# icadriani/nn_conformer_for_speech_recognition

Measured on AMD Instinct MI355X. Metric: mel-frames/sec/GPU Conformer-L encoder fwd+bwd; 1/2/4/8-GPU scaling, higher is better.
Workload: dtype bf16; 1 GPU; Conformer-L encoder fwd+bwd + CTC head, 32 x 15 s utterances per GPU; model=Conformer-L, layers=17, d_model=512, heads=8, ffn=2048, conv_kernel=31, pos_enc=none, specaug=False, global_batch=32, seq_len=1501, enc_frames=373, frontend=frame, optimizer=adafactor, parallelism=dp1, launch=hip-graph (fwd+bwd), grad_reduce_dtype=fp32

## Files before the change

### include/cfm.h

```cpp
#ifndef CFM_H
#define CFM_H

#include <stddef.h>
#include <stdint.h>

#ifdef __cplusplus
extern "C" {
#endif

#define CFM_F32 0
#define CFM_BF16 1
#define CFM_FP8 2

#define CFM_OK 0
#define CFM_ERR_ARG (-1)
#define CFM_ERR_SHAPE (-2)
#define CFM_ERR_DTYPE (-3)
#define CFM_ERR_ALIGN (-4)
#define CFM_ERR_UNSUPPORTED (-5)
#define CFM_ERR_LAUNCH (-6)

#define CFM_ACT_NONE 0
#define CFM_ACT_SILU 1

// ... 218 lines not shown
int cfm_bn_silu_bwd(const void* dz, int dtype_dz, const float* y, const float* gamma,
                    const float* beta, const float* mean, const float* invstd, int training,
                    float* dy, float* dgamma, float* dbeta, long M, int C, float* ws, void* stream);
int cfm_bn_silu_fwd_sums(const float* ws, int B, int T, int C, float* sums, void* stream);
int cfm_bn_silu_fwd_apply(const float* y, const float* gamma, const float* beta, float* running_mean,
                          float* running_var, float momentum, float eps, const float* sums, long M_total, float* mean,
                          float* invstd, void* z, int dtz, long M, int C, void* stream);
int cfm_bn_silu_bwd_sums(const void* dz, int dtdz, const float* y, const float* gamma, const float* beta,
                         const float* mean, const float* invstd, long M, int C, float* ws, float* dbeta, float* dgamma,
                         void* stream);
int cfm_bn_silu_bwd_apply(const void* dz, int dtdz, const float* y, const float* gamma, const float* beta,
                          const float* mean, const float* invstd, const float* dbeta_total, const float* dgamma_total,
                          long M_total, float* dy, long M, int C, void* stream);
size_t cfm_bn_ws_bytes(int C);
int cfm_bn_fwd(const float* y, const float* gamma, const float* beta, float* running_mean,
               float* running_var, float momentum, float eps, int training, float* mean, float* invstd,
               void* z, int dtype_z, long M, int C, int act, float* ws, void* stream);
int cfm_bn_bwd(const void* dz, int dtype_dz, const float* y, const float* gamma, const float* beta,
               const float* mean, const float* invstd, int training, int act, float* dy, float* dgamma,
               float* dbeta, long M, int C, float* ws, void* stream);
int cfm_glu_dwconv_bwd(const float* dy, const void* a, int dtype_a, const float* w_dw, void* da,
                       int dtype_da, float* dw, float* db, int B, int T, int C, int K, float* ws,
                       void* stream);
int cfm_glu_dwconv_bwd_wgrad(float* ws, int B, int T, int C, int K, float* dw, float* db, void* stream);
int cfm_glu_dwconv_bwd_bn(const void* dz, int dtype_dz, const float* y, const float* gamma, const float* beta,
                          const float* mean, const float* invstd, const float* dbeta, const float* dgamma,
                          float invM, int training, const void* a, int dtype_a, const float* w_dw, void* da,
                          int dtype_da, float* dw, float* db, int B, int T, int C, int K, float* ws, void* stream);
int cfm_gn_silu_fwd(const float* y, const float* gamma, const float* beta, float eps, float* mean, float* rstd,
                    void* z, int dtype_z, int B, int T, int C, const float* ws, void* stream);
int cfm_gn_silu_bwd_sums(const void* dz, int dtype_dz, const float* y, const float* gamma, const float* beta,
                         const float* mean, const float* rstd, int B, int T, int C, float* ws, float* dbeta,
                         float* dgamma, float* coef, void* stream);
int cfm_glu_dwconv_bwd_gn(const void* dz, int dtype_dz, const float* y, const float* gamma, const float* beta,
                          const float* mean, const float* rstd, const float* coef, const void* a, int dtype_a,
                          const float* w_dw, void* da, int dtype_da, float* dw, float* db, int B, int T, int C, int K,
                          float* ws, void* stream);
int cfm_gn_silu_bwd(const void* dz, int dtype_dz, const float* y, const float* gamma, const float* beta,
                    const float* mean, const float* rstd, float* dy, float* dgamma, float* dbeta, float* coef,
                    int B, int T, int C, float* ws, void* stream);

enum cfm_convmod_op {
  CFM_CONVMOD_OP_FWD = 0,
  CFM_CONVMOD_OP_BWD = 1,
  CFM_CONVMOD_OP_BWD_BN = 2,
  CFM_CONVMOD_OP_BWD_GN = 3
};
enum cfm_convmod_family {
  CFM_CONVMOD_FAM_UNSUPPORTED = 0,
  CFM_CONVMOD_FAM_VEC = 1,
  CFM_CONVMOD_FAM_SCALAR_KT = 2,
  CFM_CONVMOD_FAM_SCALAR_KRT = 3
};
enum cfm_convmod_apply {
  CFM_CONVMOD_APPLY_NONE = 0,
  CFM_CONVMOD_APPLY_SCALAR = 1,
  CFM_CONVMOD_APPLY_VEC8 = 2
};
typedef struct {
  int op;
  int norm;
  int dtype_a, dtype_da, dtype_dz, dtype_z;
  long M;
  int C, K;
  const void* y;
  const void* z;
  int force_scalar;
} cfm_convmod_query;
typedef struct {
  int family;
  int dz16;
  int apply;
} cfm_convmod_choice;
int cfm_convmod_plan(const cfm_convmod_query* q, cfm_convmod_choice* out);

enum cfm_attn_mode {
  CFM_ATTN_MODE_TILED = 1 << 0,
  CFM_ATTN_MODE_STAGING_ONLY = 1 << 1,
  CFM_ATTN_MODE_SKIP_STORES = 1 << 2,
  CFM_ATTN_MODE_REL_SIMT = 1 << 4,
  CFM_ATTN_MODE_REL_ZERO_FILL = 1 << 6,
  CFM_ATTN_MODE_REL_DPOS_R4 = 1 << 7,
  CFM_ATTN_MODE_REL_DQ_RECOMPUTE = 1 << 9,
  CFM_ATTN_MODE_DQ_RECOMPUTE = 1 << 10
};
int cfm_attn_set_mode(int mode);

enum cfm_attn_path {
  CFM_ATTN_PATH_SIMT = 0,
  CFM_ATTN_PATH_HEAD = 1,
  CFM_ATTN_PATH_TILED = 2,
  CFM_ATTN_PATH_REL = 3
};
enum cfm_attn_dpos {
  CFM_ATTN_DPOS_NONE = 0,
  CFM_ATTN_DPOS_XCD = 1,
  CFM_ATTN_DPOS_R4_VEC = 2,
  CFM_ATTN_DPOS_R4 = 3
};
enum cfm_attn_ws {
  CFM_ATTN_WS_D = 0,
  CFM_ATTN_WS_PART = 1,
  CFM_ATTN_WS_DS = 2,
  CFM_ATTN_WS_DPOS = 3
};
typedef struct {
  int B, T, H, dk, dtype;
  int rel;
  int qkv_mod16, dout_mod16, pos_mod16;
  int mode;
  int cus;
  int64_t ws_bytes;
} cfm_attn_query;
typedef struct {
  int path;
  int vec, vec4;
  int pvec, rel_vec;
  int dbg;
  int qs, waves;
  int dq_stored;
  int dpos;
  size_t lds_head, lds_dkdv, lds_dqs;
  size_t ws_off[4], ws_size[4];
  size_t ws_total;
} cfm_attn_choice;
int cfm_attn_plan(const cfm_attn_query* q, cfm_attn_choice* out);

int cfm_attn_fwd(const void* qkv, void* o, float* lse, const int32_t* lengths, const void* pos,
                 const float* pos_u, const float* pos_v, int B, int T, int H, int dk, int dtype,
                 float drop_p, uint64_t seed, void* stream);
size_t cfm_attn_bwd_ws_bytes(int B, int T, int H, int dk, int rel, int dtype);
int cfm_attn_bwd(const void* qkv, const void* o, const void* dout, const float* lse,
                 const int32_t* lengths, const void* pos, const float* pos_u, const float* pos_v,
                 void* dqkv, float* dpos, float* dpos_u, float* dpos_v, int B, int T, int H,
                 int dk, int dtype, float drop_p, uint64_t seed, float* ws, size_t ws_bytes, void* stream);
int cfm_attn_bwd_ex(const void* qkv, const void* o, const void* dout, const float* lse,
                    const int32_t* lengths, const void* pos, const float* pos_u, const float* pos_v,
                    void* dqkv, void* dpos, int dtype_dpos, float* dpos_u, float* dpos_v, int B, int T,
                    int H, int dk, int dtype, float drop_p, uint64_t seed, int d_ready, float* ws,
                    size_t ws_bytes, void* stream);

int cfm_conv1_fwd(const float* x, const float* w1, const float* b1, void* h1, int dtype_h, int B,
                  int F, int T, int C1, void* stream);
int cfm_conv2_fwd(const void* h1, const void* w2r, const float* b2, void* h2, int dtype_h2,
                  int dtype, int B, int F1, int T1, int C1, int C2, void* stream);
int cfm_conv2_bwd_data(const void* dh2, const void* w2r, void* dh1, int dtype, int B, int F1,
                       int T1, int C1, int C2, void* stream);
size_t cfm_conv2_bwd_data_ws_bytes(int C1, int C2);
int cfm_conv2_bwd_data_ws(const void* dh2, const void* w2r, void* dh1, int dtype, int B, int F1,
                          int T1, int C1, int C2, void* ws, void* stream);
int cfm_conv2_bwd_weight(const void* dh2, const void* h1, float* dw2r, int dtype, int B, int F1,
                         int T1, int C1, int C2, void* stream);
size_t cfm_conv2_bwd_weight_ws_bytes(int B, int F1, int T1, int C1, int C2);
int cfm_conv2_bwd_weight_ws(const void* dh2, const void* h1, float* dw2r, int dtype, int B, int F1,
                            int T1, int C1, int C2, float* ws, void* stream);
size_t cfm_conv1_bwd_ws_bytes(int B, int F, int T, int C1);
int cfm_conv1_bwd_weight(const void* dh1, int dtype_h, const float* x, float* dw1, float* db1,
                         int B, int F, int T, int C1, float* ws, void* stream);

typedef struct {
  int B, F, T;
  int C1, C2, D;
  int k1, s1, k2, s2;
  int dtype;
  int hilo;
  int F2, T2, Ke, Se, Fp, Cx, Kp, lda, T2p, Tslot;
  long xt_elems;
// ... 95 lines not shown
```

### nn_conformer_for_speech_recognition_amd/_lib.py

```python
from __future__ import annotations

import ctypes
import os
import subprocess

import torch

_HERE = os.path.dirname(os.path.abspath(__file__))
LIB_PATH = os.environ.get("CFM_LIB") or os.path.join(_HERE, "libcfm.so")
CSRC = os.path.join(_HERE, "csrc")

F32, BF16, FP8 = 0, 1, 2
ACT_NONE, ACT_SILU = 0, 1

c_void_p, c_int, c_long, c_float, c_size_t = ctypes.c_void_p, ctypes.c_int, ctypes.c_long, ctypes.c_float, ctypes.c_size_t
c_u64 = ctypes.c_uint64


class NGramLMDesc(ctypes.Structure):
    _fields_ = [("unigrams", c_void_p), ("table", c_void_p), ("seed", c_u64), ("mask", ctypes.c_uint32),
                ("probe", c_int), ("order", c_int), ("V", c_int)]


class GemmDesc(ctypes.Structure):
    _fields_ = [
        ("M", c_int), ("N", c_int), ("K", c_int), ("batch", c_int),
        ("dtype_ab", c_int),
        ("A", c_void_p), ("lda", c_long), ("stride_a", c_long), ("a_kmajor", c_int),
        ("B", c_void_p), ("ldb", c_long), ("stride_b", c_long), ("b_kmajor", c_int),
        ("C", c_void_p), ("ldc", c_long), ("stride_c", c_long), ("dtype_c", c_int),
        ("alpha", c_float),
        ("bias", c_void_p),
        ("act", c_int),
        ("act_grad", c_int),
        ("pre", c_void_p), ("dtype_pre", c_int),
        ("drop_p", c_float), ("drop_seed", c_u64), ("drop_offset", c_u64),
        ("out_scale", c_float),
        ("residual", c_void_p), ("ldr", c_long), ("dtype_r", c_int),
        ("split_k", c_int),
        ("workspace", c_void_p),
        ("probe", c_void_p),
        ("a_colsum", c_void_p),
        ("rowdot_with", c_void_p), ("rowdot_out", c_void_p), ("rowdot_T", c_int),
        ("alpha_a_dev", c_void_p), ("alpha_b_dev", c_void_p),
        ("allow_overlap", c_int),
        ("mx_a", c_void_p), ("mx_b", c_void_p),
        ("mx_out", c_void_p), ("mx_out_scales", c_void_p),
    ]


class GemmChoice(ctypes.Structure):
    _fields_ = [("variant", c_int), ("epilogue", c_int), ("grid_x", ctypes.c_uint), ("grid_y", ctypes.c_uint),
                ("grid_z", ctypes.c_uint), ("block", ctypes.c_uint)]


GEMM_MODE_STAGED256 = 1 << 0
GEMM_MODE_PIPE = 1 << 1
GEMM_MODE_DEFAULT = 3
GEMM_MODE_SKIP_STORES = 1 << 3
GEMM_MODE_SEL_SHIFT = 4
GEMM_MODE_SEL_MASK = 7 << 4
GEMM_MODE_GENERIC_DROPOUT = 1 << 10
GEMM_MODE_NO_192S8_RULE = 1 << 12
GEMM_MODE_SKIP_MAINLOOP = 1 << 13
GEMM_MODE_GENERIC_EPILOGUE = 1 << 14
GEMM_MODE_KEEP_SHARED_DMA = 1 << 19
GEMM_MODE_KEEP_PIPE192 = 1 << 21
GEMM_MODE_KEEP_128WIDE = 1 << 22
GEMM_MODE_KEEP_WS192 = 1 << 23
GEMM_SEL_AUTO, GEMM_SEL_PIPE256, GEMM_SEL_PIPE256S, GEMM_SEL_192, GEMM_SEL_PIPE192S8 = 0, 1, 2, 5, 7
(GEMM_V_NONE, GEMM_V_STAGED_BF16_256, GEMM_V_STAGED_BF16_128, GEMM_V_STAGED_F32_128, GEMM_V_STAGED_F32_64,
 GEMM_V_PIPE64X160, GEMM_V_WS192, GEMM_V_WS96, GEMM_V_PIPE192, GEMM_V_PIPE192S8, GEMM_V_PIPE256, GEMM_V_PIPE256S,
 GEMM_V_FP8_192, GEMM_V_FP8_256S, GEMM_V_MX192, GEMM_V_MX256S) = range(16)
(GEMM_EPI_GENERIC, GEMM_EPI_BF16, GEMM_EPI_BF16_BIAS, GEMM_EPI_BF16_SILU, GEMM_EPI_BF16_ACTG, GEMM_EPI_BF16_RD,
 GEMM_EPI_F32, GEMM_EPI_F32_RES, GEMM_EPI_BF16_SILU_MX, GEMM_EPI_BF16_RES, GEMM_EPI_F32R_BF16,
 GEMM_EPI_BF16_DELTA) = range(12)
CONVMOD_OP_FWD, CONVMOD_OP_BWD, CONVMOD_OP_BWD_BN, CONVMOD_OP_BWD_GN = range(4)
CONVMOD_FAM_UNSUPPORTED, CONVMOD_FAM_VEC, CONVMOD_FAM_SCALAR_KT, CONVMOD_FAM_SCALAR_KRT = range(4)
CONVMOD_APPLY_NONE, CONVMOD_APPLY_SCALAR, CONVMOD_APPLY_VEC8 = range(3)
ATTN_MODE_TILED = 1 << 0
ATTN_MODE_STAGING_ONLY = 1 << 1
ATTN_MODE_SKIP_STORES = 1 << 2
ATTN_MODE_REL_SIMT = 1 << 4
ATTN_MODE_REL_ZERO_FILL = 1 << 6
ATTN_MODE_REL_DPOS_R4 = 1 << 7
ATTN_MODE_REL_DQ_RECOMPUTE = 1 << 9
ATTN_MODE_DQ_RECOMPUTE = 1 << 10
ATTN_PATH_SIMT, ATTN_PATH_HEAD, ATTN_PATH_TILED, ATTN_PATH_REL = range(4)
ATTN_DPOS_NONE, ATTN_DPOS_XCD, ATTN_DPOS_R4_VEC, ATTN_DPOS_R4 = range(4)
ATTN_WS_D, ATTN_WS_PART, ATTN_WS_DS, ATTN_WS_DPOS = range(4)


class AttnQuery(ctypes.Structure):
    _fields_ = [(n, c_int) for n in ("B", "T", "H", "dk", "dtype", "rel", "qkv_mod16", "dout_mod16", "pos_mod16",
                                     "mode", "cus")] + [("ws_bytes", ctypes.c_int64)]


class AttnChoice(ctypes.Structure):
    _fields_ = [(n, c_int) for n in ("path", "vec", "vec4", "pvec", "rel_vec", "dbg", "qs", "waves", "dq_stored",
                                     "dpos")] + [(n, c_size_t) for n in ("lds_head", "lds_dkdv", "lds_dqs")] + [
        ("ws_off", c_size_t * 4), ("ws_size", c_size_t * 4), ("ws_total", c_size_t)]


class ConvmodQuery(ctypes.Structure):
    _fields_ = [("op", c_int), ("norm", c_int), ("dtype_a", c_int), ("dtype_da", c_int), ("dtype_dz", c_int),
                ("dtype_z", c_int), ("M", c_long), ("C", c_int), ("K", c_int), ("y", c_void_p), ("z", c_void_p),
                ("force_scalar", c_int)]


class ConvmodChoice(ctypes.Structure):
    _fields_ = [("family", c_int), ("dz16", c_int), ("apply", c_int)]


class FfoldGeo(ctypes.Structure):
    _fields_ = [(n, c_int) for n in ("B", "F", "T", "C1", "C2", "D", "k1", "s1", "k2", "s2", "dtype", "hilo",
                                     "F2", "T2", "Ke", "Se", "Fp", "Cx", "Kp", "lda", "T2p", "Tslot")] + [
        ("xt_elems", c_long), ("ws_floats", c_long)]


class AdafactorHyper(ctypes.Structure):
    _fields_ = [("decay_rate", ctypes.c_double)] + [(n, c_float) for n in (
        "lr", "beta1", "beta2t", "eps1", "eps2", "clip", "weight_decay")] + [
        ("flags", c_int), ("step_dev", c_void_p), ("scalars_dev", c_void_p)]


ADA_SCALE_PARAMETER, ADA_RELATIVE_STEP, ADA_WARMUP_INIT, ADA_DEVICE_STEP = 1, 2, 4, 8


_SIGS = {
    "cfm_version": (c_int, []),
    "cfm_get_last_error": (ctypes.c_char_p, []),
    "cfm_rng_bind": (c_int, [c_void_p]),
    "cfm_probe_slot": (c_int, [c_void_p, c_int, c_void_p]),
    "cfm_wallclock_khz": (c_int, []),
    "cfm_cast": (c_int, [c_void_p, c_int, c_void_p, c_int, c_long, c_void_p]),
    "cfm_cast_batch": (c_int, [c_void_p, c_int, c_long, c_int, c_int, c_void_p]),
    "cfm_cast_transpose_batch": (c_int, [c_void_p, c_int, c_long, c_int, c_int, c_void_p]),
    "cfm_specaug_apply": (c_int, [c_void_p, c_void_p, c_int, c_int, c_int, c_void_p, c_int, c_int, c_float, c_void_p]),
    "cfm_logmel_ws_bytes": (c_size_t, [c_int, c_int]),
    "cfm_logmel_fwd": (c_int, [c_void_p, c_long, c_void_p, c_int, c_int, c_int, c_void_p, c_void_p, c_void_p, c_void_p,
                               c_void_p, c_void_p, c_int, c_int, c_int, c_void_p, c_void_p, c_void_p]),
    "cfm_gemm": (c_int, [ctypes.POINTER(GemmDesc), c_void_p]),
    "cfm_gemm_set_mode": (c_int, [c_int]),
    "cfm_gemm_plan": (c_int, [c_void_p, c_int, c_int, c_void_p]),
    "cfm_quant_fp8": (c_int, [c_void_p, c_int, c_long, c_void_p, c_void_p, c_void_p, c_void_p]),
    "cfm_quant_fp8_ws_bytes": (c_size_t, []),
    "cfm_quant_fp8_batch_blocks": (c_long, [c_long]),
    "cfm_quant_fp8_batch": (c_int, [c_void_p, c_int, c_long, c_int, c_void_p, c_void_p]),
    "cfm_dequant_fp8": (c_int, [c_void_p, c_long, c_void_p, c_void_p, c_void_p]),
    "cfm_layernorm_fwd_mx": (c_int, [c_void_p] * 8 + [c_long, c_int, c_float, c_void_p]),
    "cfm_layernorm_fwd_mx_ex": (c_int, [c_void_p, c_int] + [c_void_p] * 7 + [c_long, c_int, c_float, c_void_p]),
    "cfm_layernorm_fwd_res": (c_int, [c_void_p, c_void_p, c_int, c_void_p, c_void_p, c_void_p, c_void_p, c_int,
                                      c_void_p, c_void_p, c_void_p, c_void_p, c_long, c_int, c_float, c_void_p]),
    "cfm_quant_mx": (c_int, [c_void_p, c_int, c_long, c_int, c_long, c_void_p, c_void_p, c_void_p]),
    "cfm_quant_mx_batch_blocks": (c_long, [c_long, c_int]),
    "cfm_quant_mx_batch": (c_int, [c_void_p, c_int, c_long, c_int, c_void_p]),
    "cfm_dequant_mx": (c_int, [c_void_p, c_void_p, c_long, c_void_p, c_void_p]),
    "cfm_wgrad_group_task_bytes": (c_size_t, []),
    "cfm_wgrad_group_tiles": (c_long, [c_int, c_int]),
    "cfm_wgrad_group_fill": (c_int, [c_void_p, c_int, c_void_p, c_void_p, c_void_p, c_void_p, c_int, c_int, c_int,
                                     c_long]),
    "cfm_wgrad_group": (c_int, [c_void_p, c_int, c_long, c_void_p]),
    "cfm_wgrad_group_probed": (c_int, [c_void_p, c_int, c_long, c_void_p, c_void_p]),
    "cfm_wgrad_group_plan": (c_long, [c_void_p, c_int, c_int, c_int, c_void_p, c_long, c_void_p]),
    "cfm_wgrad_group_ws_floats": (c_long, [c_int, c_int, c_int]),
    "cfm_wgrad_group_red_blocks": (c_long, [c_int, c_int, c_int]),
    "cfm_wgrad_group_fill_split": (c_int, [c_void_p, c_int, c_void_p, c_void_p, c_void_p, c_void_p, c_int, c_int,
                                           c_int, c_int, c_void_p, c_long]),
    "cfm_wgrad_group_sched": (c_int, [c_void_p, c_int, c_void_p, c_long, c_long, c_void_p, c_void_p]),
    "cfm_colreduce_group_task_bytes": (c_size_t, []),
# ... 203 lines not shown
```

### nn_conformer_for_speech_recognition_amd/csrc/attention.hip

```cpp
#include "attn_common.h"

namespace {

__global__ __launch_bounds__(256) void attn_fwd_kernel(AttnM p, bf16* __restrict__ o, float* __restrict__ lse) {
  if (p.drop_p > 0.f) p.seed = salted_seed(p.seed, p.salt);
  const uint32_t dkey = drop_key(p.seed, 0), dthr = drop_thr(p.drop_p);
  const float dkeep = drop_keep_scale(dthr);
  __shared__ __attribute__((aligned(16))) bf16 smem[2 * 2 * TILE * KS];
  const int tid = threadIdx.x, lane = tid & 63, wv = tid >> 6, hh = lane >> 5;
  const int h = blockIdx.y, b = blockIdx.z;
  const int q0 = blockIdx.x * 128 + wv * 32;
  const int len = p.len[b];
  const bf16* qbase = p.qkv + (long)b * p.T * p.D3 + h * p.dk;
  bf16x8 qf[4];
  load_bfrags(p, qbase, p.D3, q0 + (lane & 31), p.T, qf, lane);

  f32x16 o0 = (f32x16){0}, o1 = (f32x16){0};
  float m = -INFINITY, l = 0.f;
  const float c = p.scale * LOG2E;
  const int nkt = (len + TILE - 1) / TILE;
  uint4 rk[2], rv[2];
  const int kcol = p.HD + h * p.dk, vcol = 2 * p.HD + h * p.dk;
  if (nkt > 0) {
    tile_load(p, b, 0, kcol, rk, tid);
// ... 384 lines not shown
          }
        }
#pragma unroll
        for (int e = 0; e < 4; ++e) {
          const int r = 4 * g + e;
          const float pa = fast_exp2(__builtin_fmaf(sa[r], c, -Lr[e]));
          pf[r >> 3][r & 7] = (bf16)(pa * mk[e]);
        }
      }
      if (drop) myM[qt * 64] = (unsigned short)bits;
      if (!kvalid) pf[0] = pf[1] = (bf16x8){0};
#pragma unroll
      for (int s2 = 0; s2 < 2; ++s2) {
        dv0 = __builtin_amdgcn_mfma_f32_32x32x16_bf16(trfrag_perm(sGall, q0 + 16 * s2, 0, lane), pf[s2], dv0, 0, 0, 0);
        dv1 = __builtin_amdgcn_mfma_f32_32x32x16_bf16(trfrag_perm(sGall, q0 + 16 * s2, 32, lane), pf[s2], dv1, 0, 0, 0);
      }
    };
    f32x16 sa;
    for (int qt = 0; qt < nqs; ++qt) {
      sc(qt, sa);
      __builtin_amdgcn_sched_barrier(0);
      pdv(qt, sa);
      __builtin_amdgcn_sched_barrier(0);
    }
    store_acc_rows(dv0, dv1, 1.f, obase + 2 * p.HD, p.D3, k0w, nvalid, p.dk, v8, lane);
  }
  {
    const float keep = drop ? dkeep : 1.f;
    f32x16 dk0 = (f32x16){0}, dk1 = (f32x16){0};
    auto sg = [&](int qt, f32x16& sa, f32x16& ga) {
      sa = (f32x16){0};
      ga = (f32x16){0};
#pragma unroll
      for (int s4 = 0; s4 < 4; ++s4) {
        sa = __builtin_amdgcn_mfma_f32_32x32x16_bf16(rowfrag(sQall, qt * 32, 16 * s4, lane), kf[s4], sa, 0, 0, 0);
        ga = __builtin_amdgcn_mfma_f32_32x32x16_bf16(rowfrag(sGall, qt * 32, 16 * s4, lane), vf[s4], ga, 0, 0, 0);
      }
    };
    auto dsk = [&](int qt, const f32x16& sa, const f32x16& ga) {
      const int q0 = qt * 32;
      const unsigned bits = drop ? (unsigned)myM[qt * 64] : 0xFFFFu;
      bf16x8 sf[2];
#pragma unroll
      for (int g = 0; g < 4; ++g) {
        const float4 Lg = *reinterpret_cast<const float4*>(sL + q0 + 8 * g + 4 * hh);
        const float4 Dq = *reinterpret_cast<const float4*>(sD + q0 + 8 * g + 4 * hh);
        const float Lr[4] = {Lg.x, Lg.y, Lg.z, Lg.w}, Dr[4] = {Dq.x, Dq.y, Dq.z, Dq.w};
#pragma unroll
        for (int e = 0; e < 4; ++e) {
          const int r = 4 * g + e;
          const float pa = fast_exp2(__builtin_fmaf(sa[r], c, -Lr[e]));
          const float gk = (bits >> r) & 1u ? ga[r] : 0.f;
          sf[r >> 3][r & 7] = (bf16)(pa * __builtin_fmaf(gk, keep, -Dr[e]));
        }
      }
      if (!kvalid) sf[0] = sf[1] = (bf16x8){0};
      if (dsT) {
        bf16* drow = dsT + ((long)(b * p.H + h) * Tq + kj) * Tq + q0 + 4 * hh;
#pragma unroll
        for (int g = 0; g < 4; ++g) {
          const bf16x8& v = sf[g >> 1];
          const int o = 4 * (g & 1);
          bf16x4 w = {v[o], v[o + 1], v[o + 2], v[o + 3]};
          *reinterpret_cast<uint2*>(drow + 8 * g) = __builtin_bit_cast(uint2, w);
        }
      }
#pragma unroll
      for (int s2 = 0; s2 < 2; ++s2) {
        dk0 = __builtin_amdgcn_mfma_f32_32x32x16_bf16(trfrag_perm(sQall, q0 + 16 * s2, 0, lane), sf[s2], dk0, 0, 0, 0);
        dk1 = __builtin_amdgcn_mfma_f32_32x32x16_bf16(trfrag_perm(sQall, q0 + 16 * s2, 32, lane), sf[s2], dk1, 0, 0, 0);
      }
    };
    f32x16 sa, ga;
    for (int qt = 0; qt < nqs; ++qt) {
      sg(qt, sa, ga);
      __builtin_amdgcn_sched_barrier(0);
      dsk(qt, sa, ga);
      __builtin_amdgcn_sched_barrier(0);
    }
    store_acc_rows(dk0, dk1, p.scale, obase + p.HD, p.D3, k0w, nvalid, p.dk, v8, lane);
  }
}

__global__ __launch_bounds__(64 * HEAD_TMAX / 32) void attn_bwd_dqs_head_kernel(AttnM p, const bf16* __restrict__ dsT,
                                                                                bf16* __restrict__ dqkv) {
  extern __shared__ __attribute__((aligned(16))) bf16 hsm[];
  const int tid = threadIdx.x, lane = tid & 63, wv = tid >> 6;
  const HeadPart hp = head_part(p);
  const int b = hp.b, h = hp.h;
  const int len = p.len[b];
  const int nq = (p.T + 31) / 32, Tq = nq * 32;
  const int Tk = (p.T + TILE - 1) / TILE * TILE;
  bf16* sK = hsm;
  bf16* simg = hsm + (long)Tk * DQH_KS + wv * TILE * 32;
  const bf16* kbase = p.qkv + (long)b * p.T * p.D3 + p.HD + h * p.dk;
  for (int i = tid; i < Tk * 8; i += blockDim.x) {
    const int row = i >> 3, c = (i & 7) * 8;
    *reinterpret_cast<uint4*>(sK + row * DQH_KS + c) = ld8(kbase, p.D3, row, p.T, c, p.dk, p.vec, p.vec4);
  }
  __syncthreads();
  const int q0 = (hp.blk0 + wv) * 32;
  const int nkt = q0 < p.T ? (len + TILE - 1) / TILE : 0;
  const bf16* dbase = dsT + (long)(b * p.H + h) * Tq * Tq + (q0 < Tq ? q0 : 0);
  uint4 rd[4];
  auto dload = [&](int kt) {
#pragma unroll
    for (int i = 0; i < 4; ++i) {
      const int idx = lane + 64 * i, key = kt * TILE + (idx >> 2);
      rd[i] = key < len ? *reinterpret_cast<const uint4*>(dbase + (long)key * Tq + 8 * (idx & 3)) : make_uint4(0, 0, 0, 0);
    }
  };
  auto dstore = [&]() {
#pragma unroll
    for (int i = 0; i < 4; ++i) {
      const int idx = lane + 64 * i;
      *reinterpret_cast<uint4*>(simg + (idx >> 2) * 32 + 8 * (idx & 3)) = rd[i];
    }
  };
  f32x16 a0 = (f32x16){0}, a1 = (f32x16){0};
  if (nkt > 0) {
    dload(0);
    dstore();
  }
  for (int kt = 0; kt < nkt; ++kt) {
    if (kt + 1 < nkt) dload(kt + 1);
#pragma unroll
    for (int t = 0; t < 2; ++t)
#pragma unroll
      for (int s2 = 0; s2 < 2; ++s2) {
        const bf16x8 bfr = trfrag_perm_s<32>(simg, 32 * t + 16 * s2, 0, lane);
        const int kr = kt * TILE + 32 * t + 16 * s2;
        a0 = __builtin_amdgcn_mfma_f32_32x32x16_bf16(trfrag_perm_s<DQH_KS>(sK, kr, 0, lane), bfr, a0, 0, 0, 0);
        a1 = __builtin_amdgcn_mfma_f32_32x32x16_bf16(trfrag_perm_s<DQH_KS>(sK, kr, 32, lane), bfr, a1, 0, 0, 0);
      }
    if (kt + 1 < nkt) {
      __builtin_amdgcn_wave_barrier();
      dstore();
    }
  }
  __syncthreads();
  float* st = reinterpret_cast<float*>(hsm) + wv * 32 * 65;
  if (q0 < p.T)
    store_transposed(st, a0, a1, p.scale, dqkv + (long)b * p.T * p.D3 + h * p.dk, p.D3, q0, min(32, p.T - q0), p.dk,
                     lane);
}

__global__ __launch_bounds__(256) void attn_bwd_dot_kernel(const bf16* __restrict__ dout, const bf16* __restrict__ o,
                                                           float* __restrict__ D, int B, int T, int H, int dk) {
  __shared__ float sacc[4][1024];
  const int lane = threadIdx.x & 63, wv = threadIdx.x >> 6;
  const long row = (long)blockIdx.x * 4 + wv;
  const int HD = H * dk;
  if (row < (long)B * T) {
    const bf16* g = dout + row * HD;
    const bf16* x = o + row * HD;
    for (int c = lane; c < HD; c += 64) sacc[wv][c] = (float)g[c] * (float)x[c];
  }
  __syncthreads();
  if (row < (long)B * T) {
    const int b = (int)(row / T), t = (int)(row % T);
    for (int h = lane; h < H; h += 64) {
      float s = 0.f;
      for (int d = 0; d < dk; ++d) s += sacc[wv][h * dk + d];
      D[((long)b * H + h) * T + t] = s;
    }
  }
// ... 163 lines not shown
      s0[r] = pa * (g0[r] * ma - sLD[cur][1][qa]);
      s1[r] = pb * (g1[r] * mb - sLD[cur][1][qb]);
    }
#pragma unroll
    for (int t = 0; t < 2; ++t) {
#pragma unroll
      for (int s = 0; s < 2; ++s) {
        const bf16x8 pf = acc2frag(t == 0 ? pd0 : pd1, s);
        const bf16x8 sf = acc2frag(t == 0 ? s0 : s1, s);
        dv0 = __builtin_amdgcn_mfma_f32_32x32x16_bf16(trfrag_perm(sG, 32 * t + 16 * s, 0, lane), pf, dv0, 0, 0, 0);
        dv1 = __builtin_amdgcn_mfma_f32_32x32x16_bf16(trfrag_perm(sG, 32 * t + 16 * s, 32, lane), pf, dv1, 0, 0, 0);
        dk0 = __builtin_amdgcn_mfma_f32_32x32x16_bf16(trfrag_perm(sQ, 32 * t + 16 * s, 0, lane), sf, dk0, 0, 0, 0);
        dk1 = __builtin_amdgcn_mfma_f32_32x32x16_bf16(trfrag_perm(sQ, 32 * t + 16 * s, 32, lane), sf, dk1, 0, 0, 0);
      }
    }
    if (qt + 1 < nqt) sstore(cur ^ 1);
    __syncthreads();
  }
  float* stage = reinterpret_cast<float*>(smem) + wv * 32 * 65;
  const int nvalid = min(32, p.T - k0w);
  bf16* base = dqkv + (long)b * p.T * p.D3 + h * p.dk;
  store_transposed(stage, dk0, dk1, p.scale, base + p.HD, p.D3, k0w, nvalid, p.dk, lane);
  store_transposed(stage, dv0, dv1, 1.f, base + 2 * p.HD, p.D3, k0w, nvalid, p.dk, lane);
}


cfm_attn_query attn_query(const void* qkv, const void* dout, const void* pos, int B, int T, int H, int dk, int dtype,
                          int64_t ws_bytes) {
  return cfm_attn_query{B, T, H, dk, dtype, pos != nullptr, (int)((uintptr_t)qkv % 16), (int)((uintptr_t)dout % 16),
                        (int)((uintptr_t)pos % 16), cfm::g_attn_mode, cfm::num_cus(), ws_bytes};
}

}

namespace cfm {
int g_attn_mode = 0;
}

CFM_EXPORT int cfm_attn_set_mode(int mode) {
  cfm::g_attn_mode = mode;
  return CFM_OK;
}

CFM_EXPORT int cfm_attn_plan(const cfm_attn_query* q, cfm_attn_choice* out) {
  CFM_REQUIRE(q && out, CFM_ERR_ARG, "null pointer");
  return attn_plan(*q, *out, __func__);
}

CFM_EXPORT int cfm_attn_fwd(const void* qkv, void* o, float* lse, const int32_t* lengths, const void* pos,
                            const float* pos_u, const float* pos_v, int B, int T, int H, int dk, int dtype,
                            float drop_p, uint64_t seed, void* stream) {
  CFM_REQUIRE(qkv && o && lse && lengths, CFM_ERR_ARG, "null pointer");
  CFM_REQUIRE(!pos || (pos_u && pos_v), CFM_ERR_ARG, "rel-pos needs pos_u and pos_v");
  cfm_attn_choice c;
  if (const int rc = attn_plan(attn_query(qkv, qkv, pos, B, T, H, dk, dtype, -1), c, __func__)) return rc;
  hipStream_t s = cfm::as_stream(stream);
  if (c.path == CFM_ATTN_PATH_SIMT)
    return cfm::attn_simt_fwd_launch(qkv, o, lse, lengths, pos, pos_u, pos_v, B, T, H, dk, dtype, drop_p, seed, s);
  if (c.path == CFM_ATTN_PATH_REL)
    return cfm::attn_rel_fwd_launch(c, qkv, o, lse, lengths, pos, pos_u, pos_v, B, T, H, dk, drop_p, seed, s);
  const AttnM p = make_attnm(c, qkv, lengths, B, T, H, dk, drop_p, seed);
  if (c.path == CFM_ATTN_PATH_HEAD)
    hipLaunchKernelGGL(attn_fwd_head_kernel, dim3(B * H * c.qs), dim3(64 * c.waves), c.lds_head, s, p, (bf16*)o, lse);
  else
    hipLaunchKernelGGL(attn_fwd_kernel, dim3(cdiv(T, 128), H, B), dim3(256), 0, s, p, (bf16*)o, lse);
  return cfm::check_launch("cfm_attn_fwd");
}

CFM_EXPORT size_t cfm_attn_bwd_ws_bytes(int B, int T, int H, int dk, int rel, int dtype) {
  const cfm_attn_query q{B, T, H, dk, dtype, rel, 0, 0, 0, cfm::g_attn_mode, 1, -1};
  cfm_attn_choice c;
  return attn_plan(q, c, __func__) == CFM_OK ? c.ws_total : 0;
}

CFM_EXPORT int cfm_attn_bwd_ex(const void* qkv, const void* o, const void* dout, const float* lse,
                               const int32_t* lengths, const void* pos, const float* pos_u, const float* pos_v,
                               void* dqkv, void* dpos, int dpos_dt, float* dpos_u, float* dpos_v, int B, int T,
                               int H, int dk, int dtype, float drop_p, uint64_t seed, int d_ready, float* ws,
                               size_t ws_bytes, void* stream) {
  CFM_REQUIRE(qkv && o && dout && lse && lengths && dqkv && ws, CFM_ERR_ARG, "null pointer");
  CFM_REQUIRE(!pos || (pos_u && pos_v && dpos && dpos_u && dpos_v), CFM_ERR_ARG, "rel-pos grads need buffers");
  CFM_REQUIRE(ws_bytes <= (size_t)INT64_MAX, CFM_ERR_ARG, "ws_bytes");
  cfm_attn_choice c;
  if (const int rc = attn_plan(attn_query(qkv, dout, pos, B, T, H, dk, dtype, (int64_t)ws_bytes), c, __func__)) return rc;
  const bool mfma = c.path != CFM_ATTN_PATH_SIMT;
  CFM_REQUIRE(!d_ready || mfma, CFM_ERR_UNSUPPORTED, "precomputed D: bf16 MFMA path only");
  CFM_REQUIRE(dpos_dt == CFM_F32 || (dpos_dt == CFM_BF16 && pos && mfma), CFM_ERR_DTYPE,
              "dpos: fp32, or bf16 on the rel-pos MFMA path");
  hipStream_t s = cfm::as_stream(stream);
  if (!mfma)
    return cfm::attn_simt_bwd_launch(qkv, o, dout, lse, lengths, pos, pos_u, pos_v, dqkv, (float*)dpos, dpos_u,
                                     dpos_v, B, T, H, dk, dtype, drop_p, seed, attn_ws_ptr<float>(c, CFM_ATTN_WS_DS, ws), s);
  CFM_REQUIRE(H * dk <= 1024, CFM_ERR_UNSUPPORTED, "H*dk must be <= 1024");
  float* D = attn_ws_ptr<float>(c, CFM_ATTN_WS_D, ws);
  if (!d_ready)
    hipLaunchKernelGGL(attn_bwd_dot_kernel, dim3((unsigned)(((long)B * T + 3) / 4)), dim3(256), 0, s,
                       (const bf16*)dout, (const bf16*)o, D, B, T, H, dk);
  if (c.path == CFM_ATTN_PATH_REL)
    return cfm::attn_rel_bwd_launch(c, qkv, dout, lse, lengths, pos, pos_u, pos_v, dqkv, dpos, dpos_dt, dpos_u, dpos_v,
                                    B, T, H, dk, drop_p, seed, ws, s);
  const AttnM p = make_attnm(c, qkv, lengths, B, T, H, dk, drop_p, seed);
  if (c.path == CFM_ATTN_PATH_TILED) {
    const dim3 grid(cdiv(T, 128), H, B);
    hipLaunchKernelGGL(attn_bwd_dkdv_kernel, grid, dim3(256), 0, s, p, (const bf16*)dout, lse, D, (bf16*)dqkv);
    hipLaunchKernelGGL(attn_bwd_dq_kernel, grid, dim3(256), 0, s, p, (const bf16*)dout, lse, D, (bf16*)dqkv);
    return cfm::check_launch("cfm_attn_bwd");
  }
  const dim3 grid(B * H * c.qs), block(64 * c.waves);
  bf16* dsT = c.dq_stored ? attn_ws_ptr<bf16>(c, CFM_ATTN_WS_DS, ws) : nullptr;
  hipLaunchKernelGGL(attn_bwd_dkdv_wave_kernel, grid, block, c.lds_dkdv, s, p, (const bf16*)dout, lse, D, (bf16*)dqkv, dsT);
  if (dsT)
    hipLaunchKernelGGL(attn_bwd_dqs_head_kernel, grid, block, c.lds_dqs, s, p, (const bf16*)dsT, (bf16*)dqkv);
  else
    hipLaunchKernelGGL(attn_bwd_dq_head_kernel, grid, block, c.lds_head, s, p, (const bf16*)dout, lse, D, (bf16*)dqkv);
  return cfm::check_launch("cfm_attn_bwd");
}

CFM_EXPORT int cfm_attn_bwd(const void* qkv, const void* o, const void* dout, const float* lse,
                            const int32_t* lengths, const void* pos, const float* pos_u, const float* pos_v,
                            void* dqkv, float* dpos, float* dpos_u, float* dpos_v, int B, int T, int H, int dk,
                            int dtype, float drop_p, uint64_t seed, float* ws, size_t ws_bytes, void* stream) {
  return cfm_attn_bwd_ex(qkv, o, dout, lse, lengths, pos, pos_u, pos_v, dqkv, dpos, CFM_F32, dpos_u, dpos_v, B, T, H, dk,
                         dtype, drop_p, seed, 0, ws, ws_bytes, stream);
}
```

Baseline: 2.732 million mel-frames/s.

## Fuse dK/dV accumulation into a single sweep over query tiles in head backward

Adds a new head-path backward kernel that computes dV and dK in one pass over all query tiles, reusing the recomputed probabilities and dS per tile. The existing wave kernel, which by its name appears to do two passes, is kept behind a new DKDV_TWO_PASS mode bit, and the sweep kernel becomes the default. Dropout is split into a compile-time template so the no-dropout case skips the mask logic. The intent is to remove the second recomputation of QK^T and dO·V^T. The cost is more accumulator registers held live (four f32x16 accumulators), which may reduce occupancy.

```diff
diff --git a/include/cfm.h b/include/cfm.h
--- a/include/cfm.h
+++ b/include/cfm.h
@@ -324,7 +324,8 @@
   CFM_ATTN_MODE_REL_ZERO_FILL = 1 << 6,
   CFM_ATTN_MODE_REL_DPOS_R4 = 1 << 7,
   CFM_ATTN_MODE_REL_DQ_RECOMPUTE = 1 << 9,
-  CFM_ATTN_MODE_DQ_RECOMPUTE = 1 << 10
+  CFM_ATTN_MODE_DQ_RECOMPUTE = 1 << 10,
+  CFM_ATTN_MODE_DKDV_TWO_PASS = 1 << 11
 };
 int cfm_attn_set_mode(int mode);
 
diff --git a/nn_conformer_for_speech_recognition_amd/_lib.py b/nn_conformer_for_speech_recognition_amd/_lib.py
--- a/nn_conformer_for_speech_recognition_amd/_lib.py
+++ b/nn_conformer_for_speech_recognition_amd/_lib.py
@@ -86,6 +86,7 @@
 ATTN_MODE_REL_DPOS_R4 = 1 << 7
 ATTN_MODE_REL_DQ_RECOMPUTE = 1 << 9
 ATTN_MODE_DQ_RECOMPUTE = 1 << 10
+ATTN_MODE_DKDV_TWO_PASS = 1 << 11
 ATTN_PATH_SIMT, ATTN_PATH_HEAD, ATTN_PATH_TILED, ATTN_PATH_REL = range(4)
 ATTN_DPOS_NONE, ATTN_DPOS_XCD, ATTN_DPOS_R4_VEC, ATTN_DPOS_R4 = range(4)
 ATTN_WS_D, ATTN_WS_PART, ATTN_WS_DS, ATTN_WS_DPOS = range(4)
diff --git a/nn_conformer_for_speech_recognition_amd/csrc/attention.hip b/nn_conformer_for_speech_recognition_amd/csrc/attention.hip
--- a/nn_conformer_for_speech_recognition_amd/csrc/attention.hip
+++ b/nn_conformer_for_speech_recognition_amd/csrc/attention.hip
@@ -490,6 +490,127 @@
   }
 }
 
+template <bool DROP>
+__global__ __launch_bounds__(64 * HEAD_TMAX / 32) void attn_bwd_dkdv_sweep_kernel(AttnM p, const bf16* __restrict__ dout,
+                                                                                  const float* __restrict__ lse,
+                                                                                  const float* __restrict__ Dg,
+                                                                                  bf16* __restrict__ dqkv,
+                                                                                  bf16* __restrict__ dsT) {
+  constexpr bool drop = DROP;
+  if (drop) p.seed = salted_seed(p.seed, p.salt);
+  const uint32_t dkey = drop_key(p.seed, 0), dthr = drop_thr(p.drop_p);
+  const float dkeep = drop_keep_scale(dthr);
+  extern __shared__ __attribute__((aligned(16))) bf16 hsm[];
+  const int tid = threadIdx.x, lane = tid & 63, wv = tid >> 6, hh = lane >> 5;
+  const HeadPart hp = head_part(p);
+  const int b = hp.b, h = hp.h;
+  const int len = p.len[b];
+  const int nq = (p.T + 31) / 32, Tq = nq * 32;
+  bf16* sQall = hsm;
+  bf16* sGall = hsm + (long)Tq * KS;
+  float* sL = reinterpret_cast<float*>(sGall + (long)Tq * KS);
+  float* sD = sL + Tq;
+  const bf16* qbase = p.qkv + (long)b * p.T * p.D3 + h * p.dk;
+  head_stage(p, qbase, dout + (long)b * p.T * p.HD + h * p.dk, p.D3, p.HD, Tq, sQall, sGall, tid, blockDim.x);
+  for (int i = tid; i < Tq; i += blockDim.x) {
+    sL[i] = i < p.T ? lse[((long)b * p.H + h) * p.T + i] * LOG2E : INFINITY;
+    sD[i] = i < p.T ? Dg[((long)b * p.H + h) * p.T + i] : 0.f;
+  }
+  const int k0w = (hp.blk0 + wv) * 32;
+  const int kj = k0w + (lane & 31);
+  const bool kvalid = kj < len;
+  bf16x8 kf[4], vf[4];
+  load_bfrags(p, qbase + p.HD, p.D3, kj, p.T, kf, lane);
+  load_bfrags(p, qbase + 2 * p.HD, p.D3, kj, p.T, vf, lane);
+  __syncthreads();
+  const float c = p.scale * LOG2E;
+  const int nqs = k0w < len ? nq : 0;
+  const int odd = lane & 1, sh = 16 * odd;
+  const uint32_t T2 = (uint32_t)(p.T + (p.T & 1)) >> 1;
+  const uint32_t hbase = ((uint32_t)(b * p.H + h) * (uint32_t)p.T + (uint32_t)(4 * hh + odd)) * T2 + (uint32_t)(kj >> 1);
+  bf16* obase = dqkv + (long)b * p.T * p.D3 + h * p.dk;
+  const int nvalid = min(32, p.T - k0w);
+  const bool v8 = p.vec && ((uintptr_t)dqkv & 7) == 0;
+  const float keep = drop ? dkeep : 1.f;
+  bf16* drow0 = dsT ? dsT + ((long)(b * p.H + h) * Tq + kj) * Tq + 16 * hh : nullptr;
+
+  f32x16 dv0 = (f32x16){0}, dv1 = (f32x16){0}, dk0 = (f32x16){0}, dk1 = (f32x16){0};
+  auto sg = [&](int qt, f32x16& sa, f32x16& ga) {
+    sa = (f32x16){0};
+    ga = (f32x16){0};
+#pragma unroll
+    for (int s4 = 0; s4 < 4; ++s4)
+      sa = __builtin_amdgcn_mfma_f32_32x32x16_bf16(rowfrag(sQall, qt * 32, 16 * s4, lane), kf[s4], sa, 0, 0, 0);
+    __builtin_amdgcn_sched_barrier(0);
+#pragma unroll
+    for (int s4 = 0; s4 < 4; ++s4)
+      ga = __builtin_amdgcn_mfma_f32_32x32x16_bf16(rowfrag(sGall, qt * 32, 16 * s4, lane), vf[s4], ga, 0, 0, 0);
+  };
+  auto acc = [&](int qt, const f32x16& sa, const f32x16& ga) {
+    const int q0 = qt * 32;
+    bf16x8 pf[2], sf[2];
+#pragma unroll
+    for (int g = 0; g < 4; ++g) {
+      const float4 Lg = *reinterpret_cast<const float4*>(sL + q0 + 8 * g + 4 * hh);
+      const float4 Dq = *reinterpret_cast<const float4*>(sD + q0 + 8 * g + 4 * hh);
+      const float Lr[4] = {Lg.x, Lg.y, Lg.z, Lg.w}, Dr[4] = {Dq.x, Dq.y, Dq.z, Dq.w};
+      bool kp[4] = {true, true, true, true};
+      if (drop) {
+#pragma unroll
+        for (int e = 0; e < 4; e += 2) {
+          const uint32_t hm = attn_mix(hbase + dkey + __builtin_amdgcn_readfirstlane((q0 + 8 * g + e) * (int)T2));
+          const uint32_t ho = (uint32_t)__builtin_amdgcn_update_dpp(0, (int)hm, 0xB1, 0xF, 0xF, false);
+          const uint32_t h0 = odd ? ho : hm, h1 = odd ? hm : ho;
+          kp[e] = ((h0 >> sh) & 0xFFFFu) >= dthr;
+          kp[e + 1] = ((h1 >> sh) & 0xFFFFu) >= dthr;
+        }
+      }
+#pragma unroll
+      for (int e = 0; e < 4; ++e) {
+        const int r = 4 * g + e;
+        const float pa = fast_exp2(__builtin_fmaf(sa[r], c, -Lr[e]));
+        const float mk = drop ? (kp[e] ? dkeep : 0.f) : 1.f;
+        const float gk = kp[e] ? ga[r] : 0.f;
+        pf[r >> 3][r & 7] = (bf16)(pa * mk);
+        sf[r >> 3][r & 7] = (bf16)(pa * __builtin_fmaf(gk, keep, -Dr[e]));
+      }
+      __builtin_amdgcn_sched_barrier(0);
+    }
+    if (!kvalid) pf[0] = pf[1] = sf[0] = sf[1] = (bf16x8){0};
+#pragma unroll
+    for (int s2 = 0; s2 < 2; ++s2) {
+      dv0 = __builtin_amdgcn_mfma_f32_32x32x16_bf16(trfrag_perm(sGall, q0 + 16 * s2, 0, lane), pf[s2], dv0, 0, 0, 0);
+      dv1 = __builtin_amdgcn_mfma_f32_32x32x16_bf16(trfrag_perm(sGall, q0 + 16 * s2, 32, lane), pf[s2], dv1, 0, 0, 0);
+    }
+    __builtin_amdgcn_sched_barrier(0);
+    if (dsT) {
+      const uint4 x = __builtin_bit_cast(uint4, sf[0]), y = __builtin_bit_cast(uint4, sf[1]);
+      typedef unsigned u32x2 __attribute__((ext_vector_type(2)));
+      const u32x2 r0 = __builtin_amdgcn_permlane32_swap(x.x, y.x, false, false);
+      const u32x2 r1 = __builtin_amdgcn_permlane32_swap(x.y, y.y, false, false);
+      const u32x2 r2 = __builtin_amdgcn_permlane32_swap(x.z, y.z, false, false);
+      const u32x2 r3 = __builtin_amdgcn_permlane32_swap(x.w, y.w, false, false);
+      bf16* drow = drow0 + q0;
+      *reinterpret_cast<uint4*>(drow) = make_uint4(r0[0], r1[0], r0[1], r1[1]);
+      *reinterpret_cast<uint4*>(drow + 8) = make_uint4(r2[0], r3[0], r2[1], r3[1]);
+    }
+#pragma unroll
+    for (int s2 = 0; s2 < 2; ++s2) {
+      dk0 = __builtin_amdgcn_mfma_f32_32x32x16_bf16(trfrag_perm(sQall, q0 + 16 * s2, 0, lane), sf[s2], dk0, 0, 0, 0);
+      dk1 = __builtin_amdgcn_mfma_f32_32x32x16_bf16(trfrag_perm(sQall, q0 + 16 * s2, 32, lane), sf[s2], dk1, 0, 0, 0);
+    }
+  };
+  f32x16 sa, ga;
+  for (int qt = 0; qt < nqs; ++qt) {
+    sg(qt, sa, ga);
+    __builtin_amdgcn_sched_barrier(0);
+    acc(qt, sa, ga);
+    __builtin_amdgcn_sched_barrier(0);
+  }
+  store_acc_rows(dv0, dv1, 1.f, obase + 2 * p.HD, p.D3, k0w, nvalid, p.dk, v8, lane);
+  store_acc_rows(dk0, dk1, p.scale, obase + p.HD, p.D3, k0w, nvalid, p.dk, v8, lane);
+}
+
 __global__ __launch_bounds__(64 * HEAD_TMAX / 32) void attn_bwd_dqs_head_kernel(AttnM p, const bf16* __restrict__ dsT,
                                                                                 bf16* __restrict__ dqkv) {
   extern __shared__ __attribute__((aligned(16))) bf16 hsm[];
@@ -819,7 +940,8 @@
   CFM_REQUIRE(!pos || (pos_u && pos_v && dpos && dpos_u && dpos_v), CFM_ERR_ARG, "rel-pos grads need buffers");
   CFM_REQUIRE(ws_bytes <= (size_t)INT64_MAX, CFM_ERR_ARG, "ws_bytes");
   cfm_attn_choice c;
-  if (const int rc = attn_plan(attn_query(qkv, dout, pos, B, T, H, dk, dtype, (int64_t)ws_bytes), c, __func__)) return rc;
+  const cfm_attn_query q = attn_query(qkv, dout, pos, B, T, H, dk, dtype, (int64_t)ws_bytes);
+  if (const int rc = attn_plan(q, c, __func__)) return rc;
   const bool mfma = c.path != CFM_ATTN_PATH_SIMT;
   CFM_REQUIRE(!d_ready || mfma, CFM_ERR_UNSUPPORTED, "precomputed D: bf16 MFMA path only");
   CFM_REQUIRE(dpos_dt == CFM_F32 || (dpos_dt == CFM_BF16 && pos && mfma), CFM_ERR_DTYPE,
@@ -845,7 +967,10 @@
   }
   const dim3 grid(B * H * c.qs), block(64 * c.waves);
   bf16* dsT = c.dq_stored ? attn_ws_ptr<bf16>(c, CFM_ATTN_WS_DS, ws) : nullptr;
-  hipLaunchKernelGGL(attn_bwd_dkdv_wave_kernel, grid, block, c.lds_dkdv, s, p, (const bf16*)dout, lse, D, (bf16*)dqkv, dsT);
+  hipLaunchKernelGGL((q.mode & CFM_ATTN_MODE_DKDV_TWO_PASS) ? attn_bwd_dkdv_wave_kernel
+                     : drop_p > 0.f                          ? attn_bwd_dkdv_sweep_kernel<true>
+                                                             : attn_bwd_dkdv_sweep_kernel<false>,
+                     grid, block, c.lds_dkdv, s, p, (const bf16*)dout, lse, D, (bf16*)dqkv, dsT);
   if (dsT)
     hipLaunchKernelGGL(attn_bwd_dqs_head_kernel, grid, block, c.lds_dqs, s, p, (const bf16*)dsT, (bf16*)dqkv);
   else
```

New measurement: 2.762 million mel-frames/s, median of 6. 1.1% higher.
